# IllyaArtemchuk/Harmonies-Alphazero

Measured on AMD Instinct MI355X. Metric: self-play env-steps/sec + games/sec @4096 boards, 1/2/4/8 GPUs; bit-exact vs CPU, higher is better.
Workload: dtype u64; 1 GPU; config2: 4096 concurrent boards/GPU, reset + rule-driven play to game end (legal mask, step, chance draws, final scoring); one step = 256 hz_play launches of 4096 boards; boards_per_gpu=4096, parallelism=shard1

## Files before the change

harmonies-alphazero_amd/csrc/hz_device.hpp:

```cpp
#pragma once
#include <hip/hip_runtime.h>
#include <stdint.h>

#include "hz_initgen.hpp"

namespace hz {

constexpr int kCells = 23;
constexpr uint32_t kAll23 = (1u << 23) - 1;
constexpr int kActions = 143;
enum { WATER = 0, PLANT = 1, WOOD = 2, STONE = 3, BUILDING = 4, FIELD = 5 };
enum { PH_CHOOSE = 0, PH_P1 = 1, PH_P2 = 2, PH_P3 = 3, PH_OVER = 4 };
enum {
  ST_OK = 0, ST_BAD_PILE = 1, ST_BAD_FORMAT = 2, ST_NOT_IN_HAND = 3, ST_ILLEGAL_STACK = 4,
  ST_BAD_PHASE = 5, ST_BAD_ACTION = 6, ST_NOOP = 7
};

__host__ __device__ constexpr int initial_count(int t) {
  return t == WATER ? 23 : t == PLANT ? 19 : t == WOOD ? 21 : t == STONE ? 23 : t == BUILDING ? 15 : 19;
}

struct State {
  uint64_t pl[4];
  uint64_t piles;
// ... 511 lines not shown
#pragma unroll
    for (int u = 0; u < 8; u++) {
      uint32_t p = (prev ^ (prev >> 30)) * 1566083941U, v;
      asm("v_xad_u32 %0, %1, %2, %3" : "=v"(v) : "v"(p), "v"(cur[u]), "s"(kneg - (uint32_t)u));
      w[(g + u) * S] = v;
      prev = v;
    }
    prog(g + 8);
#pragma unroll
    for (int u = 0; u < 8; u++) cur[u] = nx[u];
  }
#pragma unroll
  for (int u = 0; u < 6; u++) {
    uint32_t v = (cur[u] ^ ((prev ^ (prev >> 30)) * 1566083941U)) - (uint32_t)(618 + u);
    w[(618 + u) * S] = v;
    prev = v;
  }
  w[1 * S] = (first1 ^ ((prev ^ (prev >> 30)) * 1566083941U)) - 1U;
  w[0] = 0x80000000U;
}

struct MTR {
  uint32_t* w;
  int stride, pos, tw;
  __device__ __forceinline__ MTR(uint32_t* words, int s, int cursor)
      : w(words), stride(s), pos(cursor & 0xFFFF), tw(cursor >> 16) {}
  __device__ __forceinline__ int cursor() const { return pos | (tw << 16); }
  __device__ __forceinline__ void prefetch() {}
  __device__ __forceinline__ uint32_t next() {
    if (pos >= kMT) { pos = 0; tw = 0; }
    if (pos >= tw) tw += twist_block(w, stride, tw);
    return temper(w[(size_t)(pos++) * stride]);
  }
};

template <class M>
__device__ __forceinline__ uint32_t randbelow(M& m, uint32_t n) {
  if (!n) return 0;
  int k = 32 - __clz(n);
  uint32_t r = m.next() >> (32 - k);
  while (r >= n) r = m.next() >> (32 - k);
  return r;
}

template <class M>
__device__ __forceinline__ void sample3_serial(M& m, uint32_t n, int k, uint32_t j[3], int got) {
  if (n <= 21) {
    for (int i = got; i < k; i++) j[i] = randbelow(m, n - (uint32_t)i);
  } else {
    for (int i = got; i < k; i++) {
      uint32_t v;
      bool dup;
      do {
        v = randbelow(m, n);
        dup = (i > 0 && j[0] == v) || (i > 1 && j[1] == v);
// ... 817 lines not shown
```

harmonies-alphazero_amd/csrc/hz_env.hip:

```cpp
#include <hip/hip_runtime.h>

#include <cstdio>
#include <cstdlib>
#include <cstring>

#include "../../include/hz_abi.h"
#include "hz_device.hpp"
#include "hz_encode.hpp"
#include "hz_host.hpp"

using namespace hz;
using namespace hz_host;

struct P2Draw {
  int32_t *tag;
  int32_t *k;
  uint64_t *q;
  uint64_t *bag;
  int32_t *c;
};
struct P2Mid {
  int32_t *tag;
  uint64_t *st;
  uint64_t *q;
// ... 37 lines not shown
  size_t nrow;
  uint32_t *ring_mt[3];
  int32_t *ring_tag[3];
  uint64_t *ring_pile[3];
  int32_t *ring_cur[3];
  int32_t *ring_k1[3];
  int calls;
  int primed, slot_valid[2];
  int32_t *mt_src;
  int lazy;
  int ar_ahead;
  uint32_t *ar_mt;
  int32_t *ar_tag;
  uint64_t *ar_pile;
  int32_t *ar_cur;
  int32_t *ar_ep[2];
  int ar_calls, ar_primed;
  uint32_t *pw_words;
  int32_t *pw_tag;
  int pipeline;
  int calls2, primed2;
  int p2_cut[kP2Play - 1];
  int p2_dcut[kP2Draw + 1];
  uint32_t *p2_s[kP2Stream];
  int32_t *p2_s_tag[kP2Stream];
  int32_t *p2_s_cur[kP2Stream];
  uint32_t *p2_p1h[2];
  int32_t *p2_p1t[2];
  uint32_t *p2_p2h[2];
  uint32_t *p2_p3h[2];
  P2Draw p2_x[kP2Draw - 1][2];
  P2Draw p2_pl[kP2Ring];
  P2Mid p2_m[kP2Play - 1][2];
  uint32_t *p2_h[kP2Ring];
  int32_t *p2_h_tag[kP2Ring];
  int32_t *p2_ep[2];
  int32_t *wait_err_own;
  int32_t *wait_err;
  int spin_limit;
};

#ifdef HZ_DIAG
__device__ uint64_t *g_stamps;
__device__ int g_role_only = -1;
#define HZ_STAMP(slot)                                                    \
  do {                                                                    \
// ... 400 lines not shown
  const int src = mt_src[b];
  if (src < kArSrc || src >= kArSrc + kArSlots) return;
  const uint32_t *from = ar_mt + ((size_t)(src - kArSrc) * n + b) * kMT;
  uint32_t *to = mt + (size_t)b * kMT;
  uint32_t v[(kMT + 63) / 64];
#pragma unroll
  for (int k = 0; k < (kMT + 63) / 64; k++) v[k] = lane + 64 * k < kMT ? from[lane + 64 * k] : 0u;
#pragma unroll
  for (int k = 0; k < (kMT + 63) / 64; k++)
    if (lane + 64 * k < kMT) to[lane + 64 * k] = v[k];
  if (lane == 0) mt_src[b] = -1;
}

static PlyWin ply_win(hz_env *e) { return PlyWin{e->pw_words, e->pw_tag, (long)e->nrow}; }

static int touch(hz_env *e) { return streams_touched<HipDev>(e) ? 0 : 1; }

static int materialize(hz_env *e) {
  if (!e->lazy) return 0;
  if (e->ar_mt)
    hipLaunchKernelGGL(k_mt_materialize_ar, dim3(e->n), dim3(64), 0, e->stream, e->mt, e->ar_mt, e->mt_src, e->n);
  hipLaunchKernelGGL(k_mt_materialize, dim3(e->n), dim3(64), 0, e->stream, e->mt, e->ahead_mt[0], e->ahead_mt[1],
                     e->mt_src, e->n);
  if (e->p2_s[0]) {
    P2Slots sl;
    for (int k = 0; k < kP2Stream; k++) sl.s[k] = e->p2_s[k];
    hipLaunchKernelGGL(k_mt_materialize2, dim3(e->n), dim3(64), 0, e->stream, e->mt, sl, e->mt_src,
                       (long)e->nrow);
  }
  e->lazy = 0;
  return launch_err();
}

static_assert(sizeof(((hz_env *)0)->p2_s) / sizeof(uint32_t *) == kP2Stream, "slot ring");

static int p2_clear_tags(hz_env *e) {
  const size_t bytes = e->nrow * sizeof(int32_t);
  auto c = [&](int32_t *t) { return hipMemsetAsync(t, 0xff, bytes, e->stream) != hipSuccess; };
  for (int k = 0; k < kP2Stream; k++)
    if (c(e->p2_s_tag[k])) return 1;
  for (int k = 0; k < 2; k++)
    if (c(e->p2_p1t[k])) return 1;
  for (int k = 0; k < kP2Draw - 1; k++)
    if (c(e->p2_x[k][0].tag) || c(e->p2_x[k][1].tag)) return 1;
  for (int k = 0; k < kP2Ring; k++)
    if (c(e->p2_pl[k].tag) || c(e->p2_h_tag[k])) return 1;
  for (int k = 0; k < kP2Play - 1; k++)
    if (c(e->p2_m[k][0].tag) || c(e->p2_m[k][1].tag)) return 1;
  return 0;
}

static int alloc_p2(hz_env *e) {
// ... 42 lines not shown
}

static int launch_play2(hz_env *e, int32_t max_plies, int32_t *games_done, int32_t *steps_done) {
  if (alloc_p2(e)) return 1;
  const int c = e->calls2, r = c & 1, w = r ^ 1;
  if (!e->primed2) {
    if (hipMemcpyAsync(e->p2_ep[w], e->episode, (size_t)e->n * sizeof(int32_t), hipMemcpyDeviceToDevice,
                       e->stream))
      return 1;
    e->primed2 = 1;
  }
  P2Args a{};
  a.st = e->state;
  a.mt = e->mt;
  a.pos = e->pos;
  a.ply = e->ply;
  a.episode = e->episode;
  a.seed = e->seed;
  a.n = e->n;
  a.max_plies = max_plies;
  a.draws = e->seed_ahead;
  a.err = e->wait_err;
  a.spin = e->spin_limit;
  for (int k = 0; k < kP2Play - 1; k++) a.cut[k] = e->p2_cut[k];
  for (int k = 0; k <= kP2Draw; k++) a.dcut[k] = e->p2_dcut[k];
  a.seed_base = e->seed_base;
  a.nrow = (long)e->nrow;
  a.games_done = games_done;
  a.steps_done = steps_done;
  a.mt_src = e->mt_src;
  a.win_tag = e->pw_tag;
  a.ep_in = e->p2_ep[w];
  a.ep_out = e->p2_ep[r];
  auto sl = [c](int s) { return ((c - s) % kP2Stream + kP2Stream) % kP2Stream; };
  for (int s = 1; s < kP2Stages; s++) {
    a.s_mt[s] = e->p2_s[sl(s)];
    a.s_tag[s] = e->p2_s_tag[sl(s)];
    a.s_cur[s] = e->p2_s_cur[sl(s)];
  }
  a.s_idx_last = sl(kP2Last);
  a.p1h_w = e->p2_p1h[r];
  a.p1h_r = e->p2_p1h[w];
  a.p1t_w = e->p2_p1t[r];
  a.p1t_r = e->p2_p1t[w];
  a.p2h_w = e->p2_p2h[r];
  a.p2h_r = e->p2_p2h[w];
// ... 13 lines not shown
    a.ht_r[st] = e->p2_h_tag[k];
  }
  for (int st = 0; st < kP2Play - 1; st++) {
    a.m_w[st] = e->p2_m[st][r];
    a.m_r[st] = e->p2_m[st][w];
  }
  const int nblk = grid_for(e->n);
  hipLaunchKernelGGL(k_play2, dim3(4 * nblk), dim3(kStageThreads), kResetLds, e->stream, a, nblk);
  if (int err = launch_err()) return err;
  e->lazy = 1;
  e->calls2 = (c + 1) % (kP2Stream * kP2Ring * 2);
  e->primed = 0;
  e->ar_primed = 0;
  return 0;
}

extern "C" {

hz_env *hz_env_create(int32_t n_boards, uint64_t seed_base, void *stream) {
  if (n_boards <= 0) return nullptr;
  if (install_comp_table()) return nullptr;
  if (lds_opt_in<k_reset>(kResetLds) || lds_opt_in<k_rollout<false, false>>(kResetLds) ||
      lds_opt_in<k_rollout<false, true>>(kResetLds) || lds_opt_in<k_rollout<true, false>>(kResetLds) ||
      lds_opt_in<k_rollout<true, true>>(kResetLds) || lds_opt_in<k_play2>(kResetLds))
    return nullptr;
  hz_env *e = new (std::nothrow) hz_env();
  if (!e) return nullptr;
  e->n = n_boards;
  e->seed_base = seed_base;
  e->stream = (hipStream_t)stream;
  const size_t n = (size_t)n_boards, nr = (n + kBlock - 1) / kBlock * kBlock, i32 = sizeof(int32_t);
  e->nrow = nr;
  DevBufs &o = e->bufs;
  o.get(e->state, n * 6 * sizeof(uint64_t), 0);
  o.get(e->mt, n * 624 * sizeof(uint32_t));
  o.get(e->pos, n * i32, 0);
  o.get(e->ply, n * i32, 0);
  o.get(e->episode, n * i32, 0);
  o.get(e->seed, n * sizeof(uint64_t), 0);
  o.get(e->mt_src, n * i32, 0xff);
  for (int k = 0; k < 2; k++) {
    o.get(e->ahead_mt[k], n * kMT * sizeof(uint32_t));
    o.get(e->ahead_tag[k], n * i32, 0xff);
    o.get(e->ahead_pile[k], n * kAheadWords * sizeof(uint64_t));
    o.get(e->ahead_cur[k], n * (kAheadDraws + 1) * i32);
    o.get(e->ahead_rule[k], nr * kRulePlies * sizeof(uint32_t));
    o.get(e->ep_final[k], n * i32);
// ... 3 lines not shown
    o.get(e->ring_tag[k], nr * i32, 0xff);
    o.get(e->ring_pile[k], nr * 3 * sizeof(uint64_t));
    o.get(e->ring_cur[k], nr * (kD1Draws + 1) * i32);
    o.get(e->ring_k1[k], nr * i32);
  }
  o.get(e->pw_words, nr * kPlyWin * sizeof(uint32_t));
  o.get(e->pw_tag, nr * i32, 0xff);
  o.get(e->wait_err_own, i32, 0);
  e->seed_ahead = kAheadDraws;
  e->ar_ahead = env_pick("HZ_AR_AHEAD", 0, 1);
  e->pipeline = env_pick("HZ_PIPELINE", 1, 2);
  for (int k = 0; k < kP2Play - 1; k++) e->p2_cut[k] = kP2PCut[k];
  if constexpr (kP2Play == 4) env_cuts("HZ_P2_CUTS", e->p2_cut);
  else if constexpr (kP2Play == 5) env_cuts_n("HZ_P2_CUTS5", e->p2_cut, kP2Play - 1, 4, 1 << 20);
  for (int k = 0; k < kP2Draw; k++) e->p2_dcut[k] = kP2DCut[k];
  e->p2_dcut[kP2Draw] = kAheadDraws;
  if constexpr (kP2Draw == 5) {
    int dc[kP2Draw + 1];
    for (int k = 0; k <= kP2Draw; k++) dc[k] = e->p2_dcut[k];
    if (env_cuts_n("HZ_P2_DCUTS", dc + 1, kP2Draw - 1, 1, kAheadDraws - 1) &&
        cuts_gaps_within(dc, kP2Draw + 1, kP2StageDraws))
      for (int k = 0; k <= kP2Draw; k++) e->p2_dcut[k] = dc[k];
  }
  e->wait_err = e->wait_err_own;
  e->spin_limit = kSpinLimitDefault;
  if (!o.ok || hipDeviceSynchronize() != hipSuccess) {
    hz_env_destroy(e);
    return nullptr;
  }
  return e;
}

void hz_env_destroy(hz_env *e) {
  if (!e) return;
  e->p2_bufs.release();
  e->ar_bufs.release();
  e->bufs.release();
  delete e;
}

int32_t hz_env_size(const hz_env *e) { return e ? e->n : -1; }

int hz_env_set_error_word(hz_env *e, int32_t *word) {
  if (!e) return -1;
  e->wait_err = word ? word : e->wait_err_own;
  return 0;
// ... 311 lines not shown
```

harmonies-alphazero_amd/csrc/hz_play2.hpp:

```cpp
#pragma once

namespace {

#ifndef HZ_P2_ST_WT
#define HZ_P2_ST_WT 0
#endif
#ifndef HZ_P2_AUX
#define HZ_P2_AUX 16
#endif
constexpr int kP2Win = 96;
constexpr int kP2WinRows = kP2Win + 24;
#ifndef HZ_P2_DCUT
#if HZ_P2_NDRAW == 5
#define HZ_P2_DCUT 0, 6, 11, 15, 19
#elif HZ_P2_NDRAW == 4
#define HZ_P2_DCUT 0, 7, 13, 18
#endif
#endif
constexpr int kP2DCut[kP2Draw] = {HZ_P2_DCUT};
constexpr int kP2StageDraws = 7;
#ifndef HZ_P2_PCUT
#if HZ_P2_NPLAY == 5
#define HZ_P2_PCUT 16, 32, 48, 64
#elif HZ_P2_NPLAY == 4
#define HZ_P2_PCUT 24, 40, 56
#endif
#endif
constexpr int kP2PCut[kP2Play - 1] = {HZ_P2_PCUT};
enum { kWvP1 = 8, kWvHash = 9, kWvPlay = 10, kWvIdle = 15 };
#ifndef HZ_P2_WAVES
#if HZ_P2_NDRAW == 5 && HZ_P2_NPLAY == 5
#define HZ_P2_WAVES 0, 1, 4, 9, 2, 3, 8, 10
// ... 48 lines not shown
  const int32_t *ep_in;
  int32_t *ep_out;
  uint32_t *s_mt[kP2Stages];
  int32_t *s_tag[kP2Stages];
  int32_t *s_cur[kP2Stages];
  int s_idx_last;
  uint32_t *p1h_w;
  const uint32_t *p1h_r;
  int32_t *p1t_w;
  const int32_t *p1t_r;
  uint32_t *p2h_w;
  const uint32_t *p2h_r;
  uint32_t *p3h_w;
  const uint32_t *p3h_r;
  P2Draw x_w[kP2Draw - 1], x_r[kP2Draw - 1];
  P2Draw pl_w, pl_r[kP2Play];
  P2Mid m_w[kP2Play - 1], m_r[kP2Play - 1];
  uint32_t *h_w;
  const uint32_t *h_r[kP2Play];
  int32_t *ht_w;
  const int32_t *ht_r[kP2Play];
  int32_t *err;
  int spin;
};

struct PlayDraw2 : PileScript {
  bool fell;
  MTR gm;
  const int32_t *cur_nd;
  __device__ __forceinline__ bool pair_pops() const { return d + 2 <= nd; }
  __device__ __forceinline__ uint32_t draw_one(uint64_t misc) {
    if (d < nd) return pop();
    if (!fell) {
      gm = MTR(gm.w, gm.stride, *cur_nd);
      fell = true;
    }
    uint32_t p9;
    return draw_pile(misc, gm, p9) ? p9 : 0x1FFu;
  }
  __device__ __forceinline__ uint32_t operator()(uint64_t misc) { return take(misc, true); }
  __device__ __forceinline__ uint32_t take(uint64_t misc, bool want) {
    if (__all(!want || d < nd)) return pop_if(want);
    return want ? draw_one(misc) : 0x1FFu;
  }
};

template <class Draw>
__device__ __forceinline__ int p2_plies(State &s, Draw &draw, int g, int g_end, uint64_t rkey, const uint32_t *hs,
                                        size_t nr) {
  const int g0 = g;
  auto hash = [&](int ply) -> uint32_t { return hs && ply < kRulePlies ? hs[(size_t)ply * nr] : rule_h32(rkey, ply); };
  const bool all_hs = __all(hs != nullptr);
  uint32_t hn[8];
  int hn_g = -1;
  while (g < g_end) {
    if (phase_of(s.misc) == PH_OVER) break;
    if (__all(g + 8 <= g_end && turn_pair_safe(s))) {
// ... 101 lines not shown
    tb = p1_load8<32>(tab, off);
    __builtin_amdgcn_sched_barrier(0);
    prev = p1_steps8(ta, prev, kA, kB);
    __builtin_amdgcn_sched_barrier(0);
    p1_arrived(tb);
    ta = p1_load8<64>(tab, off);
    __builtin_amdgcn_sched_barrier(0);
    prev = p1_steps8(tb, prev, kA, kB);
    __builtin_amdgcn_sched_barrier(0);
    p1_arrived(ta);
  }
  tb = p1_load8<0>(tab, (617 - 1) * 4);
  prev = p1_steps8(ta, prev, kA, kB);
  p1_arrived(tb);
#pragma unroll
  for (int u = 0; u < 7; u++) prev = p1_step(tb[u], prev, !(u & 1), kA, kB);
  a.p1h_w[b] = p1_step(p1_row1(kA, kB), prev, false, kA, kB);
  a.p1t_w[b] = e * 8 + 2;
}

#ifndef HZ_P2_BEND
#define HZ_P2_BEND 433
#endif
constexpr int kP2aEnd = 209, kP2bEnd = HZ_P2_BEND;
static_assert(kP2bEnd > 399 && kP2bEnd + 64 < kMT && (kP2bEnd - kAheadTwist - 1) % 8 == 0, "P2b's final steps in groups of eight; rows 397, 398 P2b's");
struct P2Ahead {
  uint32_t cur[8];
  uint32_t iv[8];
  uint32_t last;
};
typedef __attribute__((address_space(4))) const uint32_t ConstWord;
__device__ __forceinline__ ConstWord *p2_table() {
  ConstWord *t = (ConstWord *)kInitGen.v;
  asm volatile("" : "+s"(t));
  return t;
}
template <int G>
__device__ __forceinline__ void p2_ahead_init(ConstWord *tab, P2Ahead &h, uint32_t q, uint32_t kA, uint32_t kB) {
#pragma unroll
  for (int u = 0; u < 8; u++) {
    q = p1_step(tab[G + u], q, (G + u) & 1, kA, kB);
    h.cur[u] = q;
  }
#pragma unroll
  for (int u = 0; u < 8; u++) h.iv[u] = tab[G + 8 + u];
  h.last = q;
}
__device__ __forceinline__ uint32_t twist_part(uint32_t cur, uint32_t next) {
  uint32_t y;
  asm("v_bfi_b32 %0, %1, %2, %3" : "=v"(y) : "s"(0x7fffffffU), "v"(next), "v"(cur));
  return (y >> 1) ^ ((next & 1U) ? 0x9908b0dfU : 0U);
}
enum { kP2Final = 0, kP2Keep = 1, kP2Part = 2 };
typedef __attribute__((address_space(3))) uint32_t LdsWord;
struct P2Out {
  __amdgpu_buffer_rsrc_t rs;
  int row_bytes;
  int vo[8];
  uint32_t lds;
  __device__ __forceinline__ P2Out(__amdgpu_buffer_rsrc_t r, int rb, int lane) : rs(r), row_bytes(rb) {
#pragma unroll
    for (int u = 0; u < 8; u++) {
      vo[u] = lane * 4 + u * rb;
      asm volatile("" : "+v"(vo[u]));
    }
    lds = (uint32_t)(uintptr_t)(LdsWord *)(hz_lds + lane);
  }
  __device__ __forceinline__ void put(uint32_t v, int soff, int u) const {
    __builtin_amdgcn_raw_buffer_store_b32(v, rs, vo[u], soff, HZ_P2_AUX);
  }
};
template <int G0, int G1, int Mode>
__device__ __forceinline__ void p2_span(ConstWord *tab, const P2Out &o, uint32_t &prev, P2Ahead &h, uint32_t kA, uint32_t kB, int *prog) {
  constexpr bool KeepLds = Mode == kP2Keep;
  static_assert((G1 - G0) % 8 == 0, "groups of eight");
  static_assert(G1 + 15 < kMT + kInitGenPad, "the table's read-ahead within its padding");
  constexpr int S = kLdsStride;
  uint32_t lg = o.lds + G0 * S * 4;
#pragma unroll 2
  for (int g = G0; g < G1; g += 8) {
    uint32_t ivn[8], nx[8];
#pragma unroll
    for (int u = 0; u < 8; u++) ivn[u] = tab[g + 16 + u];
    const uint32_t kneg = __builtin_amdgcn_readfirstlane(0u - (uint32_t)g);
    const int soff = __builtin_amdgcn_readfirstlane((Mode == kP2Part ? g - 1 : g) * o.row_bytes);
    if (KeepLds) asm volatile("" : "+v"(lg));
    uint32_t q = h.cur[7];
#pragma unroll
    for (int u = 0; u < 8; u++) {
      const uint32_t p = (prev ^ (prev >> 30)) * 1566083941U;
      uint32_t v;
      asm("v_xad_u32 %0, %1, %2, %3" : "=v"(v) : "v"(p), "v"(h.cur[u]), "s"(kneg - (uint32_t)u));
      o.put(Mode == kP2Part ? twist_part(prev, v) : v, soff, u);
      if (KeepLds) *(LdsWord *)(uintptr_t)(lg + u * S * 4) = v;
      prev = v;
      q = p1_step(h.iv[u], q, (G0 + u) & 1, kA, kB);
      nx[u] = q;
    }
    if (KeepLds) {
      p2_publish(prog, g + 8);
      lg += 8 * S * 4;
    }
    h.last = h.cur[7];
#pragma unroll
    for (int u = 0; u < 8; u++) {
      h.cur[u] = nx[u];
      h.iv[u] = ivn[u];
    }
  }
}
template <int G, int G1, int Mode>
__device__ __forceinline__ void p2_tail(const P2Out &o, int lane, uint32_t &prev, P2Ahead &h) {
  static_assert(G1 - G >= 1 && G1 - G <= 8, "within the group ahead");
  const int soff = __builtin_amdgcn_readfirstlane((Mode == kP2Part ? G - 1 : G) * o.row_bytes);
#pragma unroll
  for (int i = G; i < G1; i++) {
    const uint32_t v = (h.cur[i - G] ^ ((prev ^ (prev >> 30)) * 1566083941U)) - (uint32_t)i;
    o.put(Mode == kP2Part ? twist_part(prev, v) : v, soff, i - G);
    if (Mode == kP2Keep) hz_lds[i * kLdsStride + lane] = v;
    prev = v;
  }
  h.last = h.cur[G1 - G - 1];
}

template <int K>
__device__ __forceinline__ void p2_third(const P2Args &a, int b0, int lane, int e, bool ok, int *s_prog) {
  const int b = b0 + lane;
  const bool act = b < a.n;
  const size_t nr = (size_t)a.nrow;
  if (K == 0 && act && !ok) a.s_tag[1][b] = -1;
  if (!__any(ok)) {
    if (K == 2) p2_publish(s_prog, kMT + 1);
    return;
  }
  uint32_t *slot = a.s_mt[1 + K];
  uint32_t kA, kB;
  p2_keys(episode_seed(a.seed_base, b, e), kA, kB);
  uint32_t prev, first1, row2, q;
  if (K == 0) {
    first1 = act ? a.p1h_r[b] : 0u;
    prev = first1;
    q = p1_row1(kA, kB);
  } else {
    const uint32_t *h = K == 1 ? a.p2h_r : a.p3h_r;
    prev = act ? h[b] : 0u;
    first1 = act ? h[nr + b] : 0u;
    row2 = act ? h[2 * nr + b] : 0u;
    q = act ? h[3 * nr + b] : 0u;
  }
  const __amdgpu_buffer_rsrc_t rs = p2_slot_rsrc(slot, b0, nr);
  const int row_bytes = __builtin_amdgcn_readfirstlane((int)(nr * 4));
  const P2Out o(rs, row_bytes, lane);
  ConstWord *tab = p2_table();
  P2Ahead h;
  if constexpr (K == 0) {
    q = p1_step(kInitGen.v[2], q, false, kA, kB);
    row2 = (q ^ ((prev ^ (prev >> 30)) * 1566083941U)) - 2U;
    prev = row2;
    p2_ahead_init<3>(tab, h, q, kA, kB);
    constexpr int G = 3 + 8 * ((kP2aEnd - 3) / 8);
    p2_span<3, G, kP2Part>(tab, o, prev, h, kA, kB, s_prog);
    p2_tail<G, kP2aEnd, kP2Part>(o, lane, prev, h);
  } else if constexpr (K == 1) {
    static_assert(kAheadTwist + 1 - kP2aEnd == 16, "P2b's part steps: two groups");
    p2_ahead_init<kP2aEnd>(tab, h, q, kA, kB);
    p2_span<kP2aEnd, kAheadTwist + 1, kP2Part>(tab, o, prev, h, kA, kB, s_prog);
    __builtin_amdgcn_raw_buffer_store_b32(prev, rs, lane * 4, kAheadTwist * row_bytes, HZ_P2_AUX);
    p2_span<kAheadTwist + 1, kP2bEnd, kP2Final>(tab, o, prev, h, kA, kB, s_prog);
  } else {
    const uint32_t f0 = act ? slot[(size_t)397 * nr + b] : 0u, f1 = act ? slot[(size_t)398 * nr + b] : 0u;
    p2_ahead_init<kP2bEnd>(tab, h, q, kA, kB);
    constexpr int G = kP2bEnd + 8 * ((kMT - kP2bEnd) / 8);
    p2_span<kP2bEnd, G, kP2Keep>(tab, o, prev, h, kA, kB, s_prog);
    p2_tail<G, kMT, kP2Keep>(o, lane, prev, h);
    p2_publish(s_prog, kMT);
    const uint32_t row1 = (first1 ^ ((prev ^ (prev >> 30)) * 1566083941U)) - 1U;
    __builtin_amdgcn_raw_buffer_store_b32(f0 ^ twist_part(0x80000000u, row1), rs, lane * 4, 0, HZ_P2_AUX);
    __builtin_amdgcn_raw_buffer_store_b32(f1 ^ twist_part(row1, row2), rs, lane * 4, row_bytes, HZ_P2_AUX);
  }
  if (K < 2) {
    if (ok) {
      uint32_t *ho = K == 0 ? a.p2h_w : a.p3h_w;
      ho[b] = prev;
      ho[nr + b] = first1;
      ho[2 * nr + b] = row2;
      ho[3 * nr + b] = h.last;
      a.s_tag[1 + K][b] = e * 8 + 3 + K;
    }
  } else if (ok) {
    a.s_tag[3][b] = e * 8 + 5;
  }
}

constexpr int kTwIters = kAheadTwist / 4;
constexpr int kTwHbm = (kP2bEnd - 397 + 3) / 4;
__device__ __forceinline__ uint4 xor4(const uint4 &a, const uint4 &b) {
  return make_uint4(a.x ^ b.x, a.y ^ b.y, a.z ^ b.z, a.w ^ b.w);
}
__device__ __forceinline__ void p2_twist(const P2Args &a, int b0, int lane, bool any, int *s_prog) {
  if (!any) return;
  const size_t nr = (size_t)a.nrow;
  uint32_t *slot = a.s_mt[3];
  const int grp = lane >> 4, c4 = (lane & 15) * 4;
  uint32_t *col = slot + b0 + c4;
  auto row = [&](int r) { return p2_ld4(col + (size_t)r * nr); };
  const __amdgpu_buffer_rsrc_t rs = p2_slot_rsrc(slot, b0, nr);
  const int row_bytes = __builtin_amdgcn_readfirstlane((int)(nr * 4));
  auto store = [&](int r, const uint4 &v) {
    typedef uint32_t v4u __attribute__((ext_vector_type(4)));
    __builtin_amdgcn_raw_buffer_store_b128(v4u{v.x, v.y, v.z, v.w}, rs, c4 * 4 + r * row_bytes, 0, HZ_P2_AUX);
  };
  [[maybe_unused]] const int b = b0 + lane;
  HZ_DIAG_T0(tz);
  int have = p2_wait(s_prog, kP2bEnd + 64, a.spin, a.err);
  P2_PHASE(35, tz);
  uint4 pt[kTwIters], fh[kTwHbm];
#pragma unroll
  for (int i = 0; i < kTwIters; i++) {
    const int r = grp + 4 * i;
    pt[i] = r >= 2 ? row(r) : make_uint4(0, 0, 0, 0);
  }
#pragma unroll
  for (int i = 0; i < kTwHbm; i++) {
    const int r = grp + 4 * i + 397;
    fh[i] = r < kP2bEnd ? row(r) : make_uint4(0, 0, 0, 0);
  }
  auto far = [&](int i) -> uint4 {
    const int r = grp + 4 * i;
    if (i < kTwHbm && r + 397 < kP2bEnd) return fh[i < kTwHbm ? i : 0];
    const uint32_t *d = hz_lds + (r + 397) * kLdsStride + c4;
    return make_uint4(d[0], d[1], d[2], d[3]);
  };
#pragma unroll
  for (int i = 0; i < kTwIters; i += 2) {
    const int need = 4 * (i + 1) + 3 + 397 + 1;
    if (need > kP2bEnd && have < need) have = p2_wait(s_prog, need, a.spin, a.err);
    const uint4 f0 = far(i), f1 = far(i + 1);
// ... 17 lines not shown
  if (w == 0) p2_third<0>(a, b0, lane, e, ok, &s_prog);
  else if (w == 1) p2_third<1>(a, b0, lane, e, ok, &s_prog);
  else if (w == 2) p2_third<2>(a, b0, lane, e, ok, &s_prog);
  else p2_twist(a, b0, lane, __any(ok), &s_prog);
}

__device__ __forceinline__ int wave_min_i(int v) {
#pragma unroll
  for (int o = 32; o > 0; o >>= 1) v = min(v, __shfl_xor(v, o));
  return v;
}
__device__ __forceinline__ void p2_draw_stage(const P2Args &a, int b0, int lane, int stage, int base) {
  const int b = b0 + lane;
  HZ_DIAG_T0(t0);
  const bool act = b < a.n;
  const size_t nr = (size_t)a.nrow;
  const int d0 = a.dcut[stage], d1 = stage == kP2Draw - 1 ? a.draws : min(a.draws, a.dcut[stage + 1]);
  const int e = act ? a.ep_in[b] + kP2Last - kP2SDraw - stage : 0;
  const uint32_t *slot = a.s_mt[kP2SDraw + stage];
  int32_t *cur = a.s_cur[kP2SDraw + stage] + b;
  const P2Draw &in = a.x_r[stage > 0 ? stage - 1 : 0];
  const P2Draw &out = stage == kP2Draw - 1 ? a.pl_w : a.x_w[stage < kP2Draw - 1 ? stage : 0];
  bool ok = act && a.s_tag[kP2SDraw + stage][b] == e * 8 + 5;
  int k0 = 0, c0 = kMTAhead;
  uint64_t bag = initial_bag(), q[kAheadWords] = {0, 0, 0, 0};
  constexpr int U = kP2Win / 4;
  const int c4 = (lane & 15) * 4;
  uint4 v[U];
  auto win_load = [&](int r0) {
#pragma unroll
    for (int u = 0; u < U; u++) {
      const int r = r0 + 4 * u + (lane >> 4);
      v[u] = p2_ld4(slot + (size_t)r * nr + b0 + c4);
    }
  };
  auto win_store = [&]() {
#pragma unroll
    for (int u = 0; u < U; u++)
      *reinterpret_cast<uint4 *>(hz_lds + base + (4 * u + (lane >> 4)) * kWinStride + c4) = v[u];
  };
  if (stage == 0) win_load(0);
  if (stage > 0 && act) {
    const int itag = in.tag[b];
    k0 = in.k[b];
    c0 = in.c[b];
    bag = in.bag[b];
#pragma unroll
    for (int i = 0; i < kAheadWords; i++) q[i] = in.q[(size_t)i * nr + b];
    ok = ok && itag == e * 8 + stage;
  }
  const bool draws = ok && k0 >= d0 && d0 < d1;
  const int r0 = wave_min_i(draws ? (c0 & 0xFFFF) : kAheadTwist) & ~3;
  if (r0 < kAheadTwist) {
    if (stage > 0) win_load(r0);
    win_store();
  }
  P2_PHASE(28 + stage, t0);
  if (!act) return;
  if (!ok) {
    out.tag[b] = -1;
    return;
  }
  if (stage == 0) cur[0] = kMTAhead;
  int k = k0, cc = c0;
  if (draws) {
    const int lim = min(r0 + kP2Win, kAheadTwist);
    StreamDraw<WinMT> d{WinMT(base - r0 * kWinStride + lane, c0, lim)};
#pragma unroll 1
    for (int i = d0; i < d1; i++) {
      if (d.m.pos >= lim) break;
      const uint32_t p9 = d(bag);
      if (d.m.pos > lim) break;
      apply_pile_fast(bag, p9);
      const int bit = 9 * i, wd = bit >> 6, off = bit & 63;
      const uint64_t lo9 = (uint64_t)p9 << off, hi9 = off > 55 ? (uint64_t)p9 >> (64 - off) : 0ull;
      q[0] |= wd == 0 ? lo9 : 0ull;
      q[1] |= wd == 1 ? lo9 : wd == 0 ? hi9 : 0ull;
      q[2] |= wd == 2 ? lo9 : wd == 1 ? hi9 : 0ull;
      q[3] |= wd == 3 ? lo9 : wd == 2 ? hi9 : 0ull;
      cc = d.m.cursor();
      p2_st(&cur[(size_t)(i + 1) * nr], cc);
      k = i + 1;
    }
  }
  p2_st(&out.k[b], k);
  p2_st(&out.c[b], cc);
  p2_st(&out.bag[b], bag);
#pragma unroll
  for (int i = 0; i < kAheadWords; i++) p2_st(&out.q[(size_t)i * nr + b], q[i]);
// ... 17 lines not shown
  } else if (code == kWvP1 && b0 + lane < a.n) {
    p2_p1(a, b0 + lane);
  } else if (code == kWvHash && b0 + lane < a.n) {
    p2_hashes(a, b0 + lane);
  }
}

__device__ __forceinline__ void p2_mid_put(const P2Mid &m, size_t nr, int b, const State &s, const PlayDraw2 &d, int g,
                                           int e) {
#pragma unroll
  for (int k = 0; k < 4; k++) p2_st(&m.st[(size_t)k * nr + b], s.pl[k]);
  p2_st(&m.st[4 * nr + b], s.piles);
  p2_st(&m.st[5 * nr + b], s.misc);
  p2_st(&m.q[b], d.q0);
  p2_st(&m.q[nr + b], d.q1);
  p2_st(&m.q[2 * nr + b], d.q2);
  p2_st(&m.q[3 * nr + b], d.q3);
  p2_st(&m.i[b], d.d);
  p2_st(&m.i[nr + b], g);
  p2_st(&m.i[2 * nr + b], d.fell ? d.gm.cursor() : -1);
  p2_st(&m.tag[b], e);
}
__device__ __forceinline__ PlayDraw2 p2_mid_get(const P2Mid &m, size_t nr, int b, State &s, int &g, int nd,
                                               uint32_t *slot, const int32_t *cur) {
#pragma unroll
  for (int k = 0; k < 4; k++) s.pl[k] = m.st[(size_t)k * nr + b];
  s.piles = m.st[4 * nr + b];
  s.misc = m.st[5 * nr + b];
  const int d = m.i[b], fc = m.i[2 * nr + b];
  g = m.i[nr + b];
  return PlayDraw2{{m.q[b], m.q[nr + b], m.q[2 * nr + b], m.q[3 * nr + b], d, nd}, fc >= 0,
                   MTR(slot, (int)nr, fc >= 0 ? fc : 0), cur + (size_t)nd * nr};
}

__device__ __forceinline__ void p2_play(const P2Args &a, int blk, int st, bool in_block) {
  __shared__ uint64_t s_lds_mask;
  const int tid = threadIdx.x, lane = tid & 63, w = tid >> 6;
  const int b0 = blk * kBlock, b = b0 + lane;
  const bool act = b < a.n;
  const uint64_t actmask = __ballot(act);
  const int nb = a.n - b0 < kBlock ? a.n - b0 : kBlock;
  const size_t nr = (size_t)a.nrow;
  HZ_DIAG_T0(t0);
  const bool last = st == kP2Play - 1;
  bool lds_used = false;
  if (act) {
    const int e = last ? a.episode[b] : a.ep_in[b] + kP2Play - 1 - st;
    const P2Draw &pl = a.pl_r[st];
    const uint32_t *hsrc = a.h_r[st];
    const int32_t *htag = a.ht_r[st];
    uint32_t *slot = a.s_mt[kP2SPlay + st] + b;
    const int32_t *cur = a.s_cur[kP2SPlay + st] + b;
    const int g_end = last ? a.max_plies : min(a.cut[st < kP2Play - 1 ? st : 0], a.max_plies);
    const uint64_t sd = episode_seed(a.seed_base, b, e), rk = rule_key(sd);
    const int ptag = pl.tag[b], nd = pl.k[b];
    const int mtag = st > 0 ? a.m_r[st - 1].tag[b] : e;
    const uint32_t *hs = htag[b] == e ? hsrc + b : nullptr;
    State s;
    int g = 0;
    PlayDraw2 draw = st == 0 ? PlayDraw2{{pl.q[b], pl.q[nr + b], pl.q[2 * nr + b], pl.q[3 * nr + b], 0, nd}, false,
                                         MTR(slot, (int)nr, 0), cur + (size_t)nd * nr}
                             : p2_mid_get(a.m_r[st - 1], nr, b, s, g, nd, slot, cur);
    const bool prep = ptag == e * 8 + kP2Draw && mtag == e;
    if (prep) {
      if (st == 0) {
        if (__all(nd >= 5)) draw.scripted_reset(s);
        else reset_state(s, draw);
      }
      P2_PHASE(16 + 2 * st, t0);
      g += p2_plies(s, draw, g, g_end, rk, hs, nr);
      P2_PHASE(17 + 2 * st, t0);
    }
    if (!last) {
      const P2Mid &mo = a.m_w[st < kP2Play - 1 ? st : 0];
      if (prep) p2_mid_put(mo, nr, b, s, draw, g, e);
      else mo.tag[b] = -1;
    } else {
      int cursor, src;
      if (prep) {
        cursor = draw.fell ? draw.gm.cursor() : cur[(size_t)draw.d * nr];
        src = 2 + a.s_idx_last;
      } else {
        mt_seed(hz_lds + lane, kLdsStride, sd);
        PlayDraw fb{{0, 0, 0, 0, 0, 0}, LdsMT(lane, kMTSeeded), false, false, MT(nullptr, 0), nullptr};
        reset_state(s, fb);
        g = p2_plies(s, fb, 0, a.max_plies, rk, nullptr, nr);
        cursor = fb.m.cursor();
        src = -1;
        lds_used = true;
      }
      a.episode[b] = e + 1;
      if (score_pending(s.misc)) finish_game(s);
      P2_PHASE(27, t0);
      store_state(a.st, a.n, b, s);
// ... 29 lines not shown
  if (g_role_only >= 0 && g_role_only != role) return;
  const uint64_t t0 = __builtin_amdgcn_s_memtime(), r0 = __builtin_amdgcn_s_memrealtime();
#endif
  if (st >= 0) p2_play(a, rb, st, role == 0);
  else if (role == 3) p2_seed(a, rb);
  else if (role != 0) p2_draw(a, rb, code);
#ifdef HZ_DIAG
  {
    const int w = threadIdx.x >> 6, bb = rb * kBlock + (threadIdx.x & 63);
    const bool idle = (role == 1 || role == 2) && code == kWvIdle;
    if (g_stamps && role > 0 && !idle && bb < a.n) g_stamps[(size_t)bb * kP2Stamps + 4 * role + w] = __builtin_amdgcn_s_memtime() - t0;
    if (g_stamps && bb < a.n && (threadIdx.x & 63) < 4) {
      const int k = threadIdx.x & 63;
      const uint64_t v = k == 0 ? r0 : k == 1 ? __builtin_amdgcn_s_memrealtime() : k == 2 ? t0 : __builtin_amdgcn_s_memtime();
      g_stamps[(size_t)(rb * kBlock + 16 * role + 4 * w + k) * kP2Stamps + 40] = v;
      if (k == 0)
        g_stamps[(size_t)(rb * kBlock + 16 * role + 4 * w) * kP2Stamps + 41] =
            (uint64_t)__builtin_amdgcn_s_getreg((31 << 11) | 4) | ((uint64_t)__builtin_amdgcn_s_getreg((15 << 11) | 20) << 32);
    }
  }
#endif
}

struct P2Slots {
  uint32_t *s[kP2Stream];
};
__global__ void __launch_bounds__(64) k_mt_materialize2(uint32_t *__restrict__ mt, P2Slots slots,
                                                       int32_t *__restrict__ mt_src, long nrow) {
  const int b = blockIdx.x, lane = threadIdx.x;
  const int src = mt_src[b];
  if (src < 2 || src >= 2 + kP2Stream) return;
  const uint32_t *from = slots.s[src - 2] + b;
  uint32_t *to = mt + (size_t)b * kMT;
  uint32_t v[(kMT + 63) / 64];
#pragma unroll
  for (int k = 0; k < (kMT + 63) / 64; k++) v[k] = lane + 64 * k < kMT ? from[(size_t)(lane + 64 * k) * nrow] : 0u;
#pragma unroll
  for (int k = 0; k < (kMT + 63) / 64; k++)
    if (lane + 64 * k < kMT) to[lane + 64 * k] = v[k];
  if (lane == 0) mt_src[b] = -1;
}


}
```

Baseline: 22.86 billion env-steps/s.

## Stop storing the full Mersenne Twister table; regenerate it from the seed when needed

By default a new lean mode has the play2 pipeline write to HBM only the first kP2Twist (160) twisted rows of each board's Mersenne Twister table, plus the final rows. The later rows are kept only in LDS or not written at all. Play-stage draws past that limit now return placeholder values and mark the board as lost, so it falls back to the existing from-seed recompute path. The materialize kernel no longer copies the slot's full table. It re-seeds and twists each affected board in LDS, then stages the result out. The draw window is also loaded at a fixed row. The aim is to cut HBM store traffic and copy bandwidth, at the price of recomputing when a board overruns the limit and when the table is materialized.

```diff
diff --git a/harmonies-alphazero_amd/csrc/hz_device.hpp b/harmonies-alphazero_amd/csrc/hz_device.hpp
--- a/harmonies-alphazero_amd/csrc/hz_device.hpp
+++ b/harmonies-alphazero_amd/csrc/hz_device.hpp
@@ -557,15 +557,15 @@
 
 struct MTR {
   uint32_t* w;
-  int stride, pos, tw;
-  __device__ __forceinline__ MTR(uint32_t* words, int s, int cursor)
-      : w(words), stride(s), pos(cursor & 0xFFFF), tw(cursor >> 16) {}
+  int stride, pos, tw, lim;
+  __device__ __forceinline__ MTR(uint32_t* words, int s, int cursor, int limit)
+      : w(words), stride(s), pos(cursor & 0xFFFF), tw(cursor >> 16), lim(limit) {}
   __device__ __forceinline__ int cursor() const { return pos | (tw << 16); }
+  __device__ __forceinline__ bool over() const { return pos > lim; }
   __device__ __forceinline__ void prefetch() {}
   __device__ __forceinline__ uint32_t next() {
-    if (pos >= kMT) { pos = 0; tw = 0; }
-    if (pos >= tw) tw += twist_block(w, stride, tw);
-    return temper(w[(size_t)(pos++) * stride]);
+    const int i = pos++;
+    return i < lim ? temper(w[(size_t)i * stride]) : 0x9E3779B9u * (uint32_t)(i + 1);
   }
 };
 
diff --git a/harmonies-alphazero_amd/csrc/hz_env.hip b/harmonies-alphazero_amd/csrc/hz_env.hip
--- a/harmonies-alphazero_amd/csrc/hz_env.hip
+++ b/harmonies-alphazero_amd/csrc/hz_env.hip
@@ -83,6 +83,7 @@
   int calls2, primed2;
   int p2_cut[kP2Play - 1];
   int p2_dcut[kP2Draw + 1];
+  int p2_fell_lim;
   uint32_t *p2_s[kP2Stream];
   int32_t *p2_s_tag[kP2Stream];
   int32_t *p2_s_cur[kP2Stream];
@@ -529,12 +530,9 @@
     hipLaunchKernelGGL(k_mt_materialize_ar, dim3(e->n), dim3(64), 0, e->stream, e->mt, e->ar_mt, e->mt_src, e->n);
   hipLaunchKernelGGL(k_mt_materialize, dim3(e->n), dim3(64), 0, e->stream, e->mt, e->ahead_mt[0], e->ahead_mt[1],
                      e->mt_src, e->n);
-  if (e->p2_s[0]) {
-    P2Slots sl;
-    for (int k = 0; k < kP2Stream; k++) sl.s[k] = e->p2_s[k];
-    hipLaunchKernelGGL(k_mt_materialize2, dim3(e->n), dim3(64), 0, e->stream, e->mt, sl, e->mt_src,
-                       (long)e->nrow);
-  }
+  if (e->p2_s[0])
+    hipLaunchKernelGGL(k_mt_materialize2, dim3(grid_for(e->n)), dim3(kStageThreads), kResetLds, e->stream, e->mt,
+                       e->seed, e->pos, e->mt_src, e->n);
   e->lazy = 0;
   return launch_err();
 }
@@ -623,6 +621,7 @@
   a.draws = e->seed_ahead;
   a.err = e->wait_err;
   a.spin = e->spin_limit;
+  a.fell_lim = e->p2_fell_lim;
   for (int k = 0; k < kP2Play - 1; k++) a.cut[k] = e->p2_cut[k];
   for (int k = 0; k <= kP2Draw; k++) a.dcut[k] = e->p2_dcut[k];
   a.seed_base = e->seed_base;
@@ -682,7 +681,8 @@
   if (install_comp_table()) return nullptr;
   if (lds_opt_in<k_reset>(kResetLds) || lds_opt_in<k_rollout<false, false>>(kResetLds) ||
       lds_opt_in<k_rollout<false, true>>(kResetLds) || lds_opt_in<k_rollout<true, false>>(kResetLds) ||
-      lds_opt_in<k_rollout<true, true>>(kResetLds) || lds_opt_in<k_play2>(kResetLds))
+      lds_opt_in<k_rollout<true, true>>(kResetLds) || lds_opt_in<k_play2>(kResetLds) ||
+      lds_opt_in<k_mt_materialize2>(kResetLds))
     return nullptr;
   hz_env *e = new (std::nothrow) hz_env();
   if (!e) return nullptr;
@@ -732,6 +732,7 @@
         cuts_gaps_within(dc, kP2Draw + 1, kP2StageDraws))
       for (int k = 0; k <= kP2Draw; k++) e->p2_dcut[k] = dc[k];
   }
+  e->p2_fell_lim = env_clamped("HZ_P2_FELL_LIMIT", kP2Twist, 0, kP2Twist);
   e->wait_err = e->wait_err_own;
   e->spin_limit = kSpinLimitDefault;
   if (!o.ok || hipDeviceSynchronize() != hipSuccess) {
diff --git a/harmonies-alphazero_amd/csrc/hz_play2.hpp b/harmonies-alphazero_amd/csrc/hz_play2.hpp
--- a/harmonies-alphazero_amd/csrc/hz_play2.hpp
+++ b/harmonies-alphazero_amd/csrc/hz_play2.hpp
@@ -8,6 +8,11 @@
 #ifndef HZ_P2_AUX
 #define HZ_P2_AUX 16
 #endif
+#ifndef HZ_P2_STATIC_WIN
+#define HZ_P2_STATIC_WIN 1
+#endif
+constexpr bool kP2StaticWin = HZ_P2_STATIC_WIN;
+
 constexpr int kP2Win = 96;
 constexpr int kP2WinRows = kP2Win + 24;
 #ifndef HZ_P2_DCUT
@@ -102,6 +107,7 @@
   const int32_t *ht_r[kP2Play];
   int32_t *err;
   int spin;
+  int fell_lim;
 };
 
 struct PlayDraw2 : PileScript {
@@ -109,10 +115,11 @@
   MTR gm;
   const int32_t *cur_nd;
   __device__ __forceinline__ bool pair_pops() const { return d + 2 <= nd; }
+  __device__ __forceinline__ bool lost() const { return fell && gm.over(); }
   __device__ __forceinline__ uint32_t draw_one(uint64_t misc) {
     if (d < nd) return pop();
     if (!fell) {
-      gm = MTR(gm.w, gm.stride, *cur_nd);
+      gm = MTR(gm.w, gm.stride, *cur_nd, gm.lim);
       fell = true;
     }
     uint32_t p9;
@@ -260,8 +267,25 @@
 #ifndef HZ_P2_BEND
 #define HZ_P2_BEND 433
 #endif
-constexpr int kP2aEnd = 209, kP2bEnd = HZ_P2_BEND;
+#ifndef HZ_P2_AEND
+#define HZ_P2_AEND 209
+#endif
+#ifndef HZ_P2_LEAN
+#define HZ_P2_LEAN 1
+#endif
+#ifndef HZ_P2_TWIST
+#define HZ_P2_TWIST 160
+#endif
+constexpr int kP2Twist = HZ_P2_TWIST;
+constexpr int kP2Ahead = 0 | (kP2Twist << 16);
+static_assert(kP2Twist % 8 == 0 && kP2Twist >= 64 && kP2Twist <= kAheadTwist, "the slot's twisted rows");
+constexpr int kP2PartEnd = HZ_P2_LEAN ? kP2Twist + 1 : kAheadTwist + 1;
+constexpr int p2_up8(int from, int x) { return x <= from ? from : from + 8 * ((x - from + 7) / 8); }
+constexpr int p2_min(int a, int b) { return a < b ? a : b; }
+constexpr int kP2aEnd = HZ_P2_AEND, kP2bEnd = HZ_P2_BEND;
 static_assert(kP2bEnd > 399 && kP2bEnd + 64 < kMT && (kP2bEnd - kAheadTwist - 1) % 8 == 0, "P2b's final steps in groups of eight; rows 397, 398 P2b's");
+static_assert(kP2aEnd > 11 && kP2aEnd <= kAheadTwist - 7 && (kAheadTwist + 1 - kP2aEnd) % 8 == 0, "P2b's part steps in groups of eight");
+constexpr int kP2bDrop = HZ_P2_LEAN ? kAheadTwist + 1 + 8 * ((397 - kAheadTwist - 1) / 8) : kAheadTwist + 1;
 struct P2Ahead {
   uint32_t cur[8];
   uint32_t iv[8];
@@ -289,7 +313,9 @@
   asm("v_bfi_b32 %0, %1, %2, %3" : "=v"(y) : "s"(0x7fffffffU), "v"(next), "v"(cur));
   return (y >> 1) ^ ((next & 1U) ? 0x9908b0dfU : 0U);
 }
-enum { kP2Final = 0, kP2Keep = 1, kP2Part = 2 };
+enum { kP2Final = 0, kP2Keep = 1, kP2Part = 2, kP2KeepLds = 3, kP2None = 4 };
+constexpr bool p2_mode_lds(int m) { return m == kP2Keep || m == kP2KeepLds; }
+constexpr bool p2_mode_hbm(int m) { return m == kP2Final || m == kP2Keep || m == kP2Part; }
 typedef __attribute__((address_space(3))) uint32_t LdsWord;
 struct P2Out {
   __amdgpu_buffer_rsrc_t rs;
@@ -310,7 +336,7 @@
 };
 template <int G0, int G1, int Mode>
 __device__ __forceinline__ void p2_span(ConstWord *tab, const P2Out &o, uint32_t &prev, P2Ahead &h, uint32_t kA, uint32_t kB, int *prog) {
-  constexpr bool KeepLds = Mode == kP2Keep;
+  constexpr bool KeepLds = p2_mode_lds(Mode), Hbm = p2_mode_hbm(Mode);
   static_assert((G1 - G0) % 8 == 0, "groups of eight");
   static_assert(G1 + 15 < kMT + kInitGenPad, "the table's read-ahead within its padding");
   constexpr int S = kLdsStride;
@@ -321,7 +347,8 @@
 #pragma unroll
     for (int u = 0; u < 8; u++) ivn[u] = tab[g + 16 + u];
     const uint32_t kneg = __builtin_amdgcn_readfirstlane(0u - (uint32_t)g);
-    const int soff = __builtin_amdgcn_readfirstlane((Mode == kP2Part ? g - 1 : g) * o.row_bytes);
+    [[maybe_unused]] int soff = 0;
+    if constexpr (Hbm) soff = __builtin_amdgcn_readfirstlane((Mode == kP2Part ? g - 1 : g) * o.row_bytes);
     if (KeepLds) asm volatile("" : "+v"(lg));
     uint32_t q = h.cur[7];
 #pragma unroll
@@ -329,7 +356,7 @@
       const uint32_t p = (prev ^ (prev >> 30)) * 1566083941U;
       uint32_t v;
       asm("v_xad_u32 %0, %1, %2, %3" : "=v"(v) : "v"(p), "v"(h.cur[u]), "s"(kneg - (uint32_t)u));
-      o.put(Mode == kP2Part ? twist_part(prev, v) : v, soff, u);
+      if constexpr (Hbm) o.put(Mode == kP2Part ? twist_part(prev, v) : v, soff, u);
       if (KeepLds) *(LdsWord *)(uintptr_t)(lg + u * S * 4) = v;
       prev = v;
       q = p1_step(h.iv[u], q, (G0 + u) & 1, kA, kB);
@@ -350,12 +377,12 @@
 template <int G, int G1, int Mode>
 __device__ __forceinline__ void p2_tail(const P2Out &o, int lane, uint32_t &prev, P2Ahead &h) {
   static_assert(G1 - G >= 1 && G1 - G <= 8, "within the group ahead");
-  const int soff = __builtin_amdgcn_readfirstlane((Mode == kP2Part ? G - 1 : G) * o.row_bytes);
+  [[maybe_unused]] const int soff = __builtin_amdgcn_readfirstlane((Mode == kP2Part ? G - 1 : G) * o.row_bytes);
 #pragma unroll
   for (int i = G; i < G1; i++) {
     const uint32_t v = (h.cur[i - G] ^ ((prev ^ (prev >> 30)) * 1566083941U)) - (uint32_t)i;
-    o.put(Mode == kP2Part ? twist_part(prev, v) : v, soff, i - G);
-    if (Mode == kP2Keep) hz_lds[i * kLdsStride + lane] = v;
+    if constexpr (p2_mode_hbm(Mode)) o.put(Mode == kP2Part ? twist_part(prev, v) : v, soff, i - G);
+    if (p2_mode_lds(Mode)) hz_lds[i * kLdsStride + lane] = v;
     prev = v;
   }
   h.last = h.cur[G1 - G - 1];
@@ -396,21 +423,28 @@
     row2 = (q ^ ((prev ^ (prev >> 30)) * 1566083941U)) - 2U;
     prev = row2;
     p2_ahead_init<3>(tab, h, q, kA, kB);
-    constexpr int G = 3 + 8 * ((kP2aEnd - 3) / 8);
-    p2_span<3, G, kP2Part>(tab, o, prev, h, kA, kB, s_prog);
-    p2_tail<G, kP2aEnd, kP2Part>(o, lane, prev, h);
+    constexpr int G = 3 + 8 * ((kP2aEnd - 3) / 8), Gp = p2_min(G, p2_up8(3, kP2PartEnd));
+    p2_span<3, Gp, kP2Part>(tab, o, prev, h, kA, kB, s_prog);
+    p2_span<Gp, G, kP2None>(tab, o, prev, h, kA, kB, s_prog);
+    p2_tail<G, kP2aEnd, (G < kP2PartEnd ? kP2Part : kP2None)>(o, lane, prev, h);
   } else if constexpr (K == 1) {
-    static_assert(kAheadTwist + 1 - kP2aEnd == 16, "P2b's part steps: two groups");
     p2_ahead_init<kP2aEnd>(tab, h, q, kA, kB);
-    p2_span<kP2aEnd, kAheadTwist + 1, kP2Part>(tab, o, prev, h, kA, kB, s_prog);
-    __builtin_amdgcn_raw_buffer_store_b32(prev, rs, lane * 4, kAheadTwist * row_bytes, HZ_P2_AUX);
-    p2_span<kAheadTwist + 1, kP2bEnd, kP2Final>(tab, o, prev, h, kA, kB, s_prog);
+    constexpr int E1 = kAheadTwist + 1, Pb = p2_min(E1, p2_up8(kP2aEnd, kP2PartEnd));
+    p2_span<kP2aEnd, Pb, kP2Part>(tab, o, prev, h, kA, kB, s_prog);
+    p2_span<Pb, E1, kP2None>(tab, o, prev, h, kA, kB, s_prog);
+    if constexpr (!HZ_P2_LEAN)
+      __builtin_amdgcn_raw_buffer_store_b32(prev, rs, lane * 4, kAheadTwist * row_bytes, HZ_P2_AUX);
+    p2_span<E1, kP2bDrop, kP2None>(tab, o, prev, h, kA, kB, s_prog);
+    p2_span<kP2bDrop, kP2bEnd, kP2Final>(tab, o, prev, h, kA, kB, s_prog);
   } else {
     const uint32_t f0 = act ? slot[(size_t)397 * nr + b] : 0u, f1 = act ? slot[(size_t)398 * nr + b] : 0u;
     p2_ahead_init<kP2bEnd>(tab, h, q, kA, kB);
     constexpr int G = kP2bEnd + 8 * ((kMT - kP2bEnd) / 8);
-    p2_span<kP2bEnd, G, kP2Keep>(tab, o, prev, h, kA, kB, s_prog);
-    p2_tail<G, kMT, kP2Keep>(o, lane, prev, h);
+    constexpr int Keep = HZ_P2_LEAN ? kP2KeepLds : kP2Keep;
+    constexpr int Kc = HZ_P2_LEAN ? p2_min(G, p2_up8(kP2bEnd, kP2Twist + 397)) : G;
+    p2_span<kP2bEnd, Kc, Keep>(tab, o, prev, h, kA, kB, s_prog);
+    p2_span<Kc, G, kP2None>(tab, o, prev, h, kA, kB, s_prog);
+    p2_tail<G, kMT, (Kc == G ? Keep : kP2None)>(o, lane, prev, h);
     p2_publish(s_prog, kMT);
     const uint32_t row1 = (first1 ^ ((prev ^ (prev >> 30)) * 1566083941U)) - 1U;
     __builtin_amdgcn_raw_buffer_store_b32(f0 ^ twist_part(0x80000000u, row1), rs, lane * 4, 0, HZ_P2_AUX);
@@ -430,7 +464,11 @@
   }
 }
 
-constexpr int kTwIters = kAheadTwist / 4;
+#ifndef HZ_P2_TWGO
+#define HZ_P2_TWGO 64
+#endif
+constexpr int kTwGo = HZ_P2_TWGO;
+constexpr int kTwIters = kP2Twist / 4;
 constexpr int kTwHbm = (kP2bEnd - 397 + 3) / 4;
 __device__ __forceinline__ uint4 xor4(const uint4 &a, const uint4 &b) {
   return make_uint4(a.x ^ b.x, a.y ^ b.y, a.z ^ b.z, a.w ^ b.w);
@@ -450,7 +488,7 @@
   };
   [[maybe_unused]] const int b = b0 + lane;
   HZ_DIAG_T0(tz);
-  int have = p2_wait(s_prog, kP2bEnd + 64, a.spin, a.err);
+  int have = kTwGo >= 0 ? p2_wait(s_prog, kP2bEnd + kTwGo, a.spin, a.err) : 0;
   P2_PHASE(35, tz);
   uint4 pt[kTwIters], fh[kTwHbm];
 #pragma unroll
@@ -514,7 +552,7 @@
   const P2Draw &in = a.x_r[stage > 0 ? stage - 1 : 0];
   const P2Draw &out = stage == kP2Draw - 1 ? a.pl_w : a.x_w[stage < kP2Draw - 1 ? stage : 0];
   bool ok = act && a.s_tag[kP2SDraw + stage][b] == e * 8 + 5;
-  int k0 = 0, c0 = kMTAhead;
+  int k0 = 0, c0 = kP2Ahead;
   uint64_t bag = initial_bag(), q[kAheadWords] = {0, 0, 0, 0};
   constexpr int U = kP2Win / 4;
   const int c4 = (lane & 15) * 4;
@@ -531,7 +569,8 @@
     for (int u = 0; u < U; u++)
       *reinterpret_cast<uint4 *>(hz_lds + base + (4 * u + (lane >> 4)) * kWinStride + c4) = v[u];
   };
-  if (stage == 0) win_load(0);
+  const int rs = kP2StaticWin ? __builtin_amdgcn_readfirstlane((3 * d0) & ~3) : 0;
+  if (kP2StaticWin || stage == 0) win_load(rs);
   if (stage > 0 && act) {
     const int itag = in.tag[b];
     k0 = in.k[b];
@@ -541,11 +580,17 @@
     for (int i = 0; i < kAheadWords; i++) q[i] = in.q[(size_t)i * nr + b];
     ok = ok && itag == e * 8 + stage;
   }
-  const bool draws = ok && k0 >= d0 && d0 < d1;
-  const int r0 = wave_min_i(draws ? (c0 & 0xFFFF) : kAheadTwist) & ~3;
-  if (r0 < kAheadTwist) {
-    if (stage > 0) win_load(r0);
+  bool draws = ok && k0 >= d0 && d0 < d1;
+  int r0 = rs;
+  if constexpr (kP2StaticWin) {
+    draws = draws && (c0 & 0xFFFF) >= r0;
     win_store();
+  } else {
+    r0 = wave_min_i(draws ? (c0 & 0xFFFF) : kP2Twist) & ~3;
+    if (r0 < kP2Twist) {
+      if (stage > 0) win_load(r0);
+      win_store();
+    }
   }
   P2_PHASE(28 + stage, t0);
   if (!act) return;
@@ -553,10 +598,10 @@
     out.tag[b] = -1;
     return;
   }
-  if (stage == 0) cur[0] = kMTAhead;
+  if (stage == 0) cur[0] = kP2Ahead;
   int k = k0, cc = c0;
   if (draws) {
-    const int lim = min(r0 + kP2Win, kAheadTwist);
+    const int lim = min(r0 + kP2Win, kP2Twist);
     StreamDraw<WinMT> d{WinMT(base - r0 * kWinStride + lane, c0, lim)};
 #pragma unroll 1
     for (int i = d0; i < d1; i++) {
@@ -620,7 +665,7 @@
   p2_st(&m.tag[b], e);
 }
 __device__ __forceinline__ PlayDraw2 p2_mid_get(const P2Mid &m, size_t nr, int b, State &s, int &g, int nd,
-                                               uint32_t *slot, const int32_t *cur) {
+                                               uint32_t *slot, const int32_t *cur, int fell_lim) {
 #pragma unroll
   for (int k = 0; k < 4; k++) s.pl[k] = m.st[(size_t)k * nr + b];
   s.piles = m.st[4 * nr + b];
@@ -628,7 +673,7 @@
   const int d = m.i[b], fc = m.i[2 * nr + b];
   g = m.i[nr + b];
   return PlayDraw2{{m.q[b], m.q[nr + b], m.q[2 * nr + b], m.q[3 * nr + b], d, nd}, fc >= 0,
-                   MTR(slot, (int)nr, fc >= 0 ? fc : 0), cur + (size_t)nd * nr};
+                   MTR(slot, (int)nr, fc >= 0 ? fc : 0, fell_lim), cur + (size_t)nd * nr};
 }
 
 __device__ __forceinline__ void p2_play(const P2Args &a, int blk, int st, bool in_block) {
@@ -657,9 +702,9 @@
     State s;
     int g = 0;
     PlayDraw2 draw = st == 0 ? PlayDraw2{{pl.q[b], pl.q[nr + b], pl.q[2 * nr + b], pl.q[3 * nr + b], 0, nd}, false,
-                                         MTR(slot, (int)nr, 0), cur + (size_t)nd * nr}
-                             : p2_mid_get(a.m_r[st - 1], nr, b, s, g, nd, slot, cur);
-    const bool prep = ptag == e * 8 + kP2Draw && mtag == e;
+                                         MTR(slot, (int)nr, 0, a.fell_lim), cur + (size_t)nd * nr}
+                             : p2_mid_get(a.m_r[st - 1], nr, b, s, g, nd, slot, cur, a.fell_lim);
+    bool prep = ptag == e * 8 + kP2Draw && mtag == e;
     if (prep) {
       if (st == 0) {
         if (__all(nd >= 5)) draw.scripted_reset(s);
@@ -668,6 +713,7 @@
       P2_PHASE(16 + 2 * st, t0);
       g += p2_plies(s, draw, g, g_end, rk, hs, nr);
       P2_PHASE(17 + 2 * st, t0);
+      if (draw.lost()) prep = false;
     }
     if (!last) {
       const P2Mid &mo = a.m_w[st < kP2Play - 1 ? st : 0];
@@ -743,24 +789,30 @@
 #endif
 }
 
-struct P2Slots {
-  uint32_t *s[kP2Stream];
-};
-__global__ void __launch_bounds__(64) k_mt_materialize2(uint32_t *__restrict__ mt, P2Slots slots,
-                                                       int32_t *__restrict__ mt_src, long nrow) {
-  const int b = blockIdx.x, lane = threadIdx.x;
-  const int src = mt_src[b];
-  if (src < 2 || src >= 2 + kP2Stream) return;
-  const uint32_t *from = slots.s[src - 2] + b;
-  uint32_t *to = mt + (size_t)b * kMT;
-  uint32_t v[(kMT + 63) / 64];
-#pragma unroll
-  for (int k = 0; k < (kMT + 63) / 64; k++) v[k] = lane + 64 * k < kMT ? from[(size_t)(lane + 64 * k) * nrow] : 0u;
-#pragma unroll
-  for (int k = 0; k < (kMT + 63) / 64; k++)
-    if (lane + 64 * k < kMT) to[lane + 64 * k] = v[k];
-  if (lane == 0) mt_src[b] = -1;
-}
-
-
-}
+__global__ void __launch_bounds__(kStageThreads) k_mt_materialize2(uint32_t *__restrict__ mt,
+                                                                  const uint64_t *__restrict__ seed,
+                                                                  const int32_t *__restrict__ pos,
+                                                                  int32_t *__restrict__ mt_src, int n) {
+  __shared__ uint64_t s_mask;
+  const int tid = threadIdx.x, lane = tid & 63;
+  const int b0 = blockIdx.x * kBlock, b = b0 + lane;
+  const int nb = n - b0 < kBlock ? n - b0 : kBlock;
+  if (tid < 64) {
+    const int src = b < n ? mt_src[b] : -1;
+    const bool mine = src >= 2 && src < 2 + kP2Stream;
+    const uint64_t m = __ballot(mine);
+    if (lane == 0) s_mask = m;
+    if (mine) {
+      mt_seed(hz_lds + lane, kLdsStride, seed[b]);
+      LdsMT s(lane, kMTSeeded);
+      s.twist_ahead(pos[b] >> 16);
+      mt_src[b] = -1;
+    }
+  }
+  __syncthreads();
+  const uint64_t mask = s_mask;
+  if (mask) stage_mt(mt + (size_t)b0 * kMT, nb, tid, mask, false);
+}
+
+
+}
```

Result: faster. 23.69 billion env-steps/s, median of 6 (+3.6%).
